# catid/longhair

Measured on AMD Instinct MI355X. Metric: GB/s of input data encoded+decoded, device-resident, per GPU and whole node, higher is better.
Workload: dtype u8

## Files before the change

### longhair_amd/csrc/codec.cpp

```cpp
#include <hip/hip_runtime.h>

#include <algorithm>
#include <atomic>
#include <cstdio>
#include <cstdlib>
#include <cstring>
#include <map>
#include <memory>
#include <mutex>
#include <stdexcept>
#include <thread>
#include <string>
#include <vector>

#include "../../include/cauchy_256.h"
#include "../../include/cauchy_256_batch.h"
#include "field.hpp"
#include "jit.hpp"
#include "host_codec.hpp"
#include "kernels.hpp"

namespace lh {

enum { kOk = 0, kInvalid = -1, kNoDevice = -2, kHipError = -3 };
// ... 136 lines not shown
    static constexpr int kDropinSlots = 4;
    DropinSlot dropin[kDropinSlots];
    std::mutex pipe_mu;
    hipStream_t pipe_stream[3] = {nullptr, nullptr, nullptr};
    hipEvent_t pipe_meta_ev = nullptr;
    DevBuf pipe_blocks[3], pipe_out[3];
    DevBuf pipe_rows, pipe_rows0, pipe_status;
    HostPinned pipe_meta;
};

static std::mutex g_devices_mu;
static std::map<int, std::unique_ptr<Device>> g_devices;

static int current_device(Device **out) {
    int id = 0;
    int count = 0;
    if (hipGetDeviceCount(&count) != hipSuccess || count <= 0)
        return fail(kNoDevice, "longhair_amd: no HIP device available (the codec has no CPU path)");
    LH_HIP(hipGetDevice(&id));
    std::lock_guard<std::mutex> g(g_devices_mu);
    auto &slot = g_devices[id];
    if (!slot) {
        std::unique_ptr<Device> d(new Device());
        d->id = id;
        const Field &F = Field::get();
        LH_HIP(hipMalloc(&d->gf_exp, 512));
        LH_HIP(hipMalloc(&d->gf_log, 256 * sizeof(int16_t)));
        LH_HIP(hipMemcpy(d->gf_exp, F.exp, 512, hipMemcpyHostToDevice));
        LH_HIP(hipMemcpy(d->gf_log, F.log, 256 * sizeof(int16_t), hipMemcpyHostToDevice));
        LH_HIP(hipDeviceGetAttribute(&d->cus, hipDeviceAttributeMultiprocessorCount, id));
        d->jump2 = jump_table2_usable(id);
        slot = std::move(d);
    }
    *out = slot.get();
    return kOk;
}

static bool capturing(hipStream_t st) {
    hipStreamCaptureStatus cs = hipStreamCaptureStatusNone;
    if (hipStreamIsCapturing(st, &cs) != hipSuccess) {
        (void)hipGetLastError();
        return false;
    }
    return cs != hipStreamCaptureStatusNone;
}

static int capture_growth_error(const char *what) {
    return fail(kHipError, std::string("longhair_amd: the ") + what +
                               " must grow while the stream is being captured; reserve it before capture with "
                               "cauchy_256_batch_prepare_stream(k, m, bytes, max_stripes, stream) or an "
                               "uncaptured call of the same size on that stream");
}

static int device_generator(Device *d, int k, int m, const uint8_t **out, const uint8_t **points = nullptr,
                            hipStream_t st = nullptr) {
    std::lock_guard<std::mutex> g(d->mu);
    auto it = d->generators.find({k, m});
    if (it == d->generators.end()) {
        if (capturing(st)) return capture_growth_error("generator matrix");
        std::vector<uint8_t> G = generator_matrix(k, m);
        std::vector<uint8_t> xs, ys;
        const bool pts = cauchy_points(k, m, xs, ys);
        if (pts) {
            G.insert(G.end(), xs.begin(), xs.end());
            G.insert(G.end(), ys.begin(), ys.end());
        }
        uint8_t *p = nullptr;
        LH_HIP(hipMalloc(&p, G.size()));
        LH_HIP(hipMemcpy(p, G.data(), G.size(), hipMemcpyHostToDevice));
        it = d->generators.emplace(std::make_pair(k, m), std::make_pair(p, pts)).first;
    }
    *out = it->second.first;
    if (points) *points = it->second.second ? it->second.first + (size_t)k * m : nullptr;
    return kOk;
}

static int zero_page(Device *d, size_t bytes, const uint8_t **out, hipStream_t st = nullptr) {
    std::lock_guard<std::mutex> g(d->mu);
    if (d->zero.size < bytes) {
        if (capturing(st)) return capture_growth_error("zero page");
        uint8_t *p = nullptr;
        LH_HIP(hipMalloc(&p, bytes));
        LH_HIP(hipMemsetAsync(p, 0, bytes, nullptr));
        LH_HIP(hipStreamSynchronize(nullptr));
        if (d->zero.ptr) d->retired.push_back(d->zero.ptr);
        d->zero.ptr = p;
        d->zero.size = bytes;
    }
    *out = d->zero.ptr;
    return kOk;
}

static int workspace(Device *d, hipStream_t st, size_t plan_bytes, size_t work_bytes, Workspace **out) {
    std::lock_guard<std::mutex> g(d->mu);
    Workspace &w = d->ws[st];
    if ((plan_bytes > w.plan.size || work_bytes > w.work.size) && capturing(st))
        return capture_growth_error("per-stream decode workspace");
    LH_HIP(w.plan.reserve(plan_bytes, st));
    if (work_bytes) LH_HIP(w.work.reserve(work_bytes, st));
    *out = &w;
    return kOk;
}

static long long jit_blocks(const JitConfig &cfg, int stripes) {
    const long long waves = cfg.spw ? (stripes + cfg.spw - 1) / cfg.spw : (long long)stripes * cfg.wps;
    long long blocks = (waves + 3) / 4;
    return blocks;
}
static long long jit_encode_blocks(const JitConfig &cfg, int stripes) {
    const long long waves = cfg.spw ? (stripes + cfg.spw - 1) / cfg.spw : (long long)stripes * cfg.wps;
    return (waves + cfg.enc_wpb - 1) / cfg.enc_wpb;
}
static int generic_word(int sub) {
    if (sub >= 4) return 4;
    if (sub >= 2) return 2;
    return 1;
}

static const JitKernels *jit_lookup(Device *d, const JitConfig &cfg, bool allow_compile, std::string *err,
                                    bool *hard) {
    const JitMode mode = allow_compile ? batch_jit_mode() : JitMode::kCached;
    bool failed = false;
    const JitKernels *jk = d->jit.get(cfg, err, mode, &failed);
    *hard = !jk && failed && mode == JitMode::kBlocking;
    return jk;
}
// ... 111 lines not shown

enum { kFormStrided = 1, kFormFamily = 2, kFormTable = 4 };
static void shape_configs(int k, int m, int bytes, bool decode, int forms, std::vector<JitConfig> *out) {
    JitConfig cfg, c;
    if (jit_config_for(k, m, bytes, decode, &cfg)) {
        if (forms & kFormStrided) out->push_back(cfg);
        if ((forms & kFormFamily) && !cfg.family && jit_family_config_for(k, m, bytes, &c, decode)) out->push_back(c);
        if ((forms & kFormTable) && jit_ptr_config_for(k, m, bytes, decode, &c)) out->push_back(c);
    } else if (jit_win_config_for(k, m, bytes, &cfg, decode)) {
        if (forms & kFormStrided) out->push_back(cfg);
        if ((forms & kFormTable) && jit_win_ptr_config_for(k, m, bytes, &c, decode)) out->push_back(c);
    }
}

static void note_jit_launch(const char *kernel, const Route &r, const Blocks &b) {
    char name[64];
    std::snprintf(name, sizeof name, "%s%s", kernel, b.table ? "(pointer table)" : r.cfg.family ? "(family)" : "");
    note_launch(name);
}

static int launch_jit_encode(const Route &r, int bytes, int stripes, Blocks in, Blocks out, hipStream_t st) {
    long long blocks = jit_encode_blocks(r.cfg, stripes);
    if (r.cfg.family) {
        const long long spw = 64 / ((bytes / 8 + 7) / 8);
        blocks = ((stripes + spw - 1) / spw + r.cfg.enc_wpb - 1) / r.cfg.enc_wpb;
    }
    if (blocks > 0x7FFFFFFF) return fail(kInvalid, "batch too large");
    int n = stripes, bb = bytes;
    void *args[] = {(void *)&in.p, &in.stride, (void *)&out.p, &out.stride, &n, &bb};
    const unsigned lds = in.table ? 0 : r.jk->dyn_lds;
    LH_HIP(hipModuleLaunchKernel(r.jk->encode, (unsigned)blocks, 1, 1, 64u * (unsigned)r.cfg.enc_wpb, 1, 1, lds, st,
                                 args, nullptr));
    note_jit_launch("lh_jit_encode", r, in);
    return kOk;
}

static int launch_jit_encode_win(const Route &r, int m, int bytes, int stripes, Blocks in, Blocks out, hipStream_t st) {
    const long long blocks = (long long)stripes * (r.cfg.sub / (64 * r.cfg.W));
    if (blocks > 0x7FFFFFFF) return fail(kInvalid, "batch too large");
    const unsigned threads = 64u * (unsigned)((m + r.cfg.rows_per_wave - 1) / r.cfg.rows_per_wave);
    int n = stripes, bb = bytes;
    void *args[] = {(void *)&in.p, &in.stride, (void *)&out.p, &out.stride, &n, &bb};
    LH_HIP(hipModuleLaunchKernel(r.jk->encode_win, (unsigned)blocks, 1, 1, threads, 1, 1, 0, st, args, nullptr));
    note_jit_launch("lh_jit_encode_win", r, in);
    return kOk;
}

static int launch_jit_decode_fused(Device *d, const Route &r, int bytes, int stripes, Blocks blk, uint8_t *d_rows,
                                   int8_t *d_status, hipStream_t st) {
    const long long blocks = jit_blocks(r.cfg, stripes);
    if (blocks > 0x7FFFFFFF) return fail(kInvalid, "batch too large");
    const uint8_t *zero = nullptr;
    if (int rc = zero_page(d, (size_t)bytes, &zero, st)) return rc;
    const uint8_t *gexp = d->gf_exp;
    const int16_t *glog = d->gf_log;
    int n = stripes, bb = bytes;
    void *args[] = {(void *)&blk.p, &blk.stride, (void *)&d_rows, (void *)&d_status, (void *)&zero,
                    (void *)&gexp, (void *)&glog, &n, &bb};
    const unsigned lds = blk.table ? 0 : r.jk->dyn_lds;
    LH_HIP(hipModuleLaunchKernel(r.jk->decode_fused, (unsigned)blocks, 1, 1, 256, 1, 1, lds, st, args, nullptr));
    note_jit_launch("lh_jit_decode_fused", r, blk);
    return kOk;
}

static int launch_jit_decode(Device *d, const Route &r, int bytes, int stripes, Blocks blk, const Workspace *w,
                             long long plan_stride, hipStream_t st) {
    const long long blocks = jit_blocks(r.cfg, stripes);
    if (blocks > 0x7FFFFFFF) return fail(kInvalid, "batch too large");
    const uint8_t *zero = nullptr;
    if (int rc = zero_page(d, (size_t)bytes, &zero, st)) return rc;
    const uint8_t *plan = w->plan.ptr;
    int n = stripes;
    void *args[] = {(void *)&blk.p, &blk.stride, (void *)&plan, &plan_stride, (void *)&zero, &n};
    LH_HIP(hipModuleLaunchKernel(r.jk->decode, (unsigned)blocks, 1, 1, 256, 1, 1, 0, st, args, nullptr));
    note_jit_launch("lh_jit_decode", r, blk);
    return kOk;
}

static size_t plan_order_offset(int stripes, long long plan_stride) {
    return ((size_t)stripes * (size_t)plan_stride + 15) & ~(size_t)15;
}
static size_t plan_workspace_bytes(int k, int m, int e_max, int stripes) {
    return plan_order_offset(stripes, PlanView::bytes(k, m, e_max)) + (size_t)stripes * sizeof(int);
}

static int launch_jit_decode_wide(Device *d, const Route &r, int k, int m, int e_max, int bytes, int stripes,
                                  Blocks blk, const Workspace *w, long long plan_stride, hipStream_t st) {
    const long long blocks = (long long)stripes * (r.cfg.sub / (64 * r.cfg.W));
    if (blocks > 0x7FFFFFFF) return fail(kInvalid, "batch too large");
    const uint8_t *zero = nullptr;
    if (int rc = zero_page(d, (size_t)bytes, &zero, st)) return rc;
    const unsigned threads = 64u * (unsigned)((m + r.cfg.rows_per_wave - 1) / r.cfg.rows_per_wave);
    const uint8_t *plan = w->plan.ptr;
    int n = stripes, bb = bytes;
    void *args[] = {(void *)&blk.p, &blk.stride, (void *)&plan, &plan_stride, (void *)&zero, &n, &bb};
    LH_HIP(hipModuleLaunchKernel(r.jk->decode_wide, (unsigned)blocks, 1, 1, threads, 1, 1, 0, st, args, nullptr));
    note_jit_launch("lh_jit_decode_wide", r, blk);
    InverseArgs ia{};
    set_blocks(ia, blk);
    ia.plan = plan;
    ia.plan_stride = plan_stride;
    ia.k = k;
    ia.m = m;
    ia.e_max = e_max;
    ia.bytes = bytes;
    ia.stripes = stripes;
    ia.order = (int *)(w->plan.ptr + plan_order_offset(stripes, plan_stride));
    LH_HIP(launch_inverse(ia, st));
    return kOk;
}

// ... 975 lines not shown
```

### longhair_amd/csrc/jit.cpp

```cpp
#include "jit.hpp"

#include <hip/hiprtc.h>
#include <dlfcn.h>
#include <sys/stat.h>
#include <unistd.h>
#include <utime.h>

#include <algorithm>
#include <cstdio>
#include <cstdlib>
#include <cstring>
#include <deque>
#include <functional>
#include <sstream>
#include <thread>

#include "field.hpp"

extern "C" const char lh_jit_source[];
extern "C" const char lh_inv_jump_source[];

namespace lh {

namespace {
// ... 456 lines not shown
    if (c.win) {
        std::string tok;
        for (char ch : c.defines + " ") {
            if (ch == ' ' || ch == ',') {
                const size_t eq = tok.find('=');
                if (!tok.empty()) os << "#define " << (eq == std::string::npos ? tok : tok.substr(0, eq) + " " + tok.substr(eq + 1)) << "\n";
                tok.clear();
            } else {
                tok += ch;
            }
        }
        os << win_source_for(c);
        return os.str();
    }
    {
        std::string tok;
        for (char ch : c.defines + " ") {
            if (ch == ' ' || ch == ',') {
                const size_t eq = tok.find('=');
                if (!tok.empty()) os << "#define " << (eq == std::string::npos ? tok : tok.substr(0, eq) + " " + tok.substr(eq + 1)) << "\n";
                tok.clear();
            } else {
                tok += ch;
            }
        }
    }
    if (c.family) {
        os << "#define LH_FAMILY 1\n#define LH_K " << c.k << "\n#define LH_M " << c.m
           << "\n#define LH_BYTES 1024\n#define LH_SUB 128\n#define LH_W 8\n#define LH_NCH 16\n#define LH_SPW 4"
              "\n#define LH_WPS 1\n#ifndef LH_LDS\n#define LH_LDS 1\n#endif\n#ifndef LH_CPS\n#define LH_CPS "
           << c.cps << "\n#endif\n#define LH_ROLE " << c.role << "\n#define LH_DEC_PLAIN 0\n";
    } else {
    os << "#define LH_K " << c.k << "\n#define LH_M " << c.m << "\n#define LH_BYTES " << c.bytes
       << "\n#define LH_SUB " << c.sub << "\n#define LH_W " << c.W << "\n#define LH_NCH " << c.nch
       << "\n#define LH_SPW " << (c.spw ? c.spw : 1) << "\n#define LH_WPS " << (c.wps ? c.wps : 1) << "\n";
    if (c.ptr) os << "#define LH_PTR 1\n#define LH_BUF 0\n";
    if (c.lds) os << "#ifndef LH_LDS\n#define LH_LDS 1\n#endif\n";
    if (c.cps > 1 && !c.ptr) os << "#ifndef LH_CPS\n#define LH_CPS " << c.cps << "\n#endif\n";
    if (c.role) os << "#define LH_ROLE " << c.role << "\n#define LH_DEC_PLAIN " << c.plain << "\n";
    }
    const std::vector<uint8_t> g = generator_matrix(c.k, c.m);
    os << "static constexpr unsigned char LH_BM[" << c.m << "][" << c.k << "][8] = {";
    for (int r = 0; r < c.m; ++r) {
        os << "{";
        for (int x = 0; x < c.k; ++x) {
            const uint64_t bm = bitmatrix(g[(size_t)r * c.k + x]);
            os << "{";
            for (int y = 0; y < 8; ++y) os << (unsigned)((bm >> (8 * y)) & 0xFF) << (y < 7 ? "," : "");
            os << "}" << (x + 1 < c.k ? "," : "");
        }
        os << "}" << (r + 1 < c.m ? "," : "");
    }
    os << "};\n";
    os << "#define LH_G_INIT {";
    for (int r = 0; r < c.m; ++r) {
        os << "{";
        for (int x = 0; x < c.k; ++x) os << (unsigned)g[(size_t)r * c.k + x] << (x + 1 < c.k ? "," : "");
        os << "}" << (r + 1 < c.m ? "," : "");
    }
    os << "}\n";
    os << lh_jit_source;
    return os.str();
}

JitCache::Key JitCache::key_of(const JitConfig &cfg) {
    return Key(cfg.k, cfg.m, (cfg.win || cfg.family) ? 0 : cfg.bytes, cfg.W, cfg.defines + (cfg.family ? "|family" : ""),
               cfg.lds * 1000000000 + cfg.ptr * 100000000 + (cfg.role + 3 * cfg.plain) * 10000000 +
                   cfg.win_split * 1000000 + cfg.win * 100000 + cfg.win_lds * 10000 +
                   cfg.rows_per_wave * 100 + cfg.win_pf);
}

const JitKernels *JitCache::peek(const JitConfig &cfg) {
    std::lock_guard<std::mutex> g(mu_);
    auto it = cache_.find(key_of(cfg));
    return it == cache_.end() ? nullptr : &it->second;
}

static const char *kOpts[] = {"--offload-arch=gfx950", "-O3", "-std=c++17", "-mllvm", "-enable-gvn-memdep=false",
                              "-mllvm", "-enable-load-pre=false"};

static uint64_t fnv1a(const std::string &s, uint64_t h = 1469598103934665603ull) {
    for (unsigned char ch : s) h = (h ^ ch) * 1099511628211ull;
    return h;
}

static std::string cache_dir() {
    if (const char *d = std::getenv("LONGHAIR_AMD_CACHE_DIR")) return d;
    Dl_info info;
    if (dladdr((void *)&fnv1a, &info) && info.dli_fname) {
        std::string p = info.dli_fname;
        const size_t slash = p.rfind('/');
        if (slash != std::string::npos) {
            std::string d = p.substr(0, slash) + "/jit_cache";
            mkdir(d.c_str(), 0755);
            if (access(d.c_str(), W_OK) == 0) return d;
        }
    }
    if (const char *home = std::getenv("HOME")) {
        std::string d = std::string(home) + "/.cache";
        mkdir(d.c_str(), 0755);
        d += "/longhair_amd";
        mkdir(d.c_str(), 0755);
        return d;
    }
    return "";
}

static std::string cache_path(const std::string &src) {
    std::string key = src;
    for (const char *o : kOpts) key += std::string("\n") + o;
    static const std::string ver = [] {
        int major = 0, minor = 0;
        (void)hiprtcVersion(&major, &minor);
// ... 304 lines not shown
```

### longhair_amd/csrc/jit_codec.hip

```cpp

#ifndef LH_K
#define LH_K 4
#define LH_M 2
#define LH_BYTES 64
#define LH_SUB 8
#define LH_W 8
#define LH_NCH 1
#define LH_SPW 64
#define LH_WPS 0
static constexpr unsigned char LH_BM[LH_M][LH_K][8] = {
    {{1, 2, 4, 8, 16, 32, 64, 128}, {1, 2, 4, 8, 16, 32, 64, 128},
     {1, 2, 4, 8, 16, 32, 64, 128}, {1, 2, 4, 8, 16, 32, 64, 128}},
    {{1, 2, 4, 8, 16, 32, 64, 128}, {2, 4, 8, 16, 32, 64, 128, 135},
     {3, 6, 12, 24, 48, 96, 192, 7}, {4, 8, 16, 32, 64, 128, 135, 137}}};
#define LH_G_INIT {{1, 1, 1, 1}, {1, 2, 3, 4}}
#include <hip/hip_runtime.h>
#endif

#define LH_NW ((LH_W + 3) / 4)


struct lh_word {
    unsigned int v[LH_NW];
};

#ifndef LH_NT
#define LH_NT 1
#endif
typedef unsigned int lh_u32x2 __attribute__((ext_vector_type(2)));
typedef unsigned int lh_u32x3 __attribute__((ext_vector_type(3)));
typedef unsigned int lh_u32x4 __attribute__((ext_vector_type(4)));

__device__ __forceinline__ lh_word lh_load(const unsigned char *p) {
    lh_word w;
#if LH_NT && LH_W == 16
    const lh_u32x4 v = __builtin_nontemporal_load((const lh_u32x4 *)p);
    w.v[0] = v.x; w.v[1] = v.y; w.v[2] = v.z; w.v[3] = v.w;
#elif LH_NT && LH_W == 12
    const lh_u32x3 v = __builtin_nontemporal_load((const lh_u32x3 *)p);
    w.v[0] = v.x; w.v[1] = v.y; w.v[2] = v.z;
#elif LH_NT && LH_W == 8
    const lh_u32x2 v = __builtin_nontemporal_load((const lh_u32x2 *)p);
    w.v[0] = v.x; w.v[1] = v.y;
#elif LH_NT && LH_W == 4
    w.v[0] = __builtin_nontemporal_load((const unsigned int *)p);
#else
#pragma unroll
    for (int i = 0; i < LH_NW; ++i) w.v[i] = 0;
    __builtin_memcpy(&w.v[0], p, LH_W);
#endif
    return w;
}

#ifndef LH_NT_ST
#define LH_NT_ST LH_NT
#endif
#ifndef LH_BUF
#define LH_BUF 1
#endif
#ifndef LH_PTR
#define LH_PTR 0
#endif
#if LH_PTR && LH_BUF
#error "LH_PTR: scattered blocks are addressed by 64-bit pointers (LH_BUF 0)"
#endif
#ifndef LH_NT_DEC
#define LH_NT_DEC 0
#endif
// ... 1171 lines not shown

template <int PF, class PREP>
__device__ __forceinline__ void lh_decode_body(const lh_lane &l, long long wave, unsigned char *__restrict__ blocks,
                                               long long stripe_stride, lh_plan_regs &pr,
                                               const unsigned char *__restrict__ zero_page, int stripes,
                                               const PREP &prep) {
    const lh_dsrc S = lh_make_dsrc(l, wave, blocks, stripe_stride, zero_page, stripes);
    lh_word v[LH_M][8];
    {
        lh_word ring[PF][8];
        lh_dec_issue<PF>(ring, pr, S);
        prep(pr);
        lh_dec_phase_a<PF>(v, ring, pr, S);
    }
#if LH_BUF
    lh_dec_phase_b(v, pr, blocks + l.stripe * stripe_stride + l.p, l.last, S, S.lbase - l.p);
#elif LH_PTR
    lh_dec_phase_b(v, pr, nullptr, l.last, S, l.p);
#else
    lh_dec_phase_b(v, pr, blocks + l.stripe * stripe_stride + l.p, l.last, S, 0);
#endif
}

__device__ __forceinline__ void lh_decode_wave(long long wave, unsigned char *__restrict__ blocks,
                                               long long stripe_stride, const unsigned char *__restrict__ plan,
                                               long long plan_stride, const unsigned char *__restrict__ zero_page,
                                               int stripes) {
    const lh_lane l = lh_map_lane(stripes, wave);
    if (!l.active) return;
    const unsigned char *pl = plan + l.stripe * plan_stride;
    lh_plan_regs pr;
    pr.e = pl[0];
    if (pr.e == 0) return;
    lh_load_packed(pr.srcw, pl + LH_P_SRC);
    lh_load_packed(pr.recw, pl + LH_P_REC);
    lh_load_packed(pr.coefw, pl + LH_P_COEF);
    lh_load_packed(pr.outw, pl + LH_P_OUT);
    lh_decode_body<LH_PF_DEC>(l, wave, blocks, stripe_stride, pr, zero_page, stripes, lh_no_prep());
}

#if LH_ROLE == 0 || (LH_ROLE == 2 && (LH_DEC_PLAIN || !(LH_EMAX <= 4 && LH_NCH <= 64 && LH_K <= 64)))
extern "C" __global__ void __launch_bounds__(256)
lh_jit_decode(unsigned char *__restrict__ blocks, long long stripe_stride,
              const unsigned char *__restrict__ plan, long long plan_stride,
              const unsigned char *__restrict__ zero_page, int stripes) {
    LH_WAVE_LOOP(stripes) { lh_decode_wave(lh_w, blocks, stripe_stride, plan, plan_stride, zero_page, stripes); }
}
#endif

#if LH_EMAX <= 4 && LH_NCH <= 64 && LH_K <= 64
#define LH_FUSED 1
#undef LH_DWPB
#define LH_DWPB 4
static constexpr unsigned char LH_GRAW[LH_M][LH_K] = LH_G_INIT;
#define LH_P4(n) (((n) + 3) / 4 * 4)
#define LH_SR (2 * LH_P4(LH_K) + LH_P4(LH_M))
#define LH_NRW ((LH_K + LH_NCH - 1) / LH_NCH)
#define LH_STRIPE_LANES (LH_NCH >= 64 ? ~0ull : ((1ull << (LH_NCH & 63)) - 1))

struct lh_gct {
    static constexpr int nch = LH_NCH, nrw = LH_NRW, maxrw = LH_NRW;
    static constexpr unsigned long long lanes = LH_STRIPE_LANES;
};

template <class G>
__device__ __forceinline__ void lh_fused_rows(const G &g, const lh_lane &l, int c, const unsigned char *__restrict__ rows,
                                              unsigned int (&rowv)[G::maxrw]) {
    const unsigned char *grow = rows + l.stripe * LH_K;
#pragma unroll
    for (int t = 0; t < G::maxrw; ++t) {
        const int i = c + t * g.nch;
        rowv[t] = (l.active && t < g.nrw && i < LH_K) ? (unsigned int)grow[i] : 0u;
    }
}

struct lh_fused_solve {
    unsigned int rs[LH_EMAX], rr[LH_EMAX], er[LH_EMAX];
    unsigned char *grow;
    const unsigned char *gexp;
    const short *glog;
    const unsigned char *gmat;
    int c;
    __device__ __forceinline__ void operator()(lh_plan_regs &pr) const;
};

template <class G>
__device__ __forceinline__ bool lh_fused_plan(const G &g, const lh_lane &l, int c, int sl, unsigned char *scr,
                                              const unsigned int (&rowv)[G::maxrw],
                                              unsigned char *__restrict__ rows, signed char *__restrict__ status,
                                              lh_fused_solve &sv, lh_plan_regs &pr) {
    unsigned char *lrows = scr;
    unsigned char *lsrc = scr + LH_P4(LH_K);
    unsigned char *lrec = lsrc + LH_P4(LH_K);
    unsigned char *grow = rows + l.stripe * LH_K;
    for (int q = c; q < (LH_P4(LH_K) + LH_P4(LH_M)) / 4; q += g.nch) ((unsigned int *)lsrc)[q] = 0xFFFFFFFFu;
    bool bad = false;
#pragma unroll
    for (int t = 0; t < G::maxrw; ++t) {
        const int i = c + t * g.nch;
        if (t >= g.nrw || i >= LH_K) continue;
        const unsigned int r = rowv[t];
        lrows[i] = (unsigned char)r;
        if (r < LH_K) lsrc[r] = (unsigned char)i;
        else if (r < LH_K + LH_M) lrec[r - LH_K] = (unsigned char)i;
        else bad = true;
    }
    for (int i = c; i < LH_K; i += g.nch) {
        const unsigned int r = lrows[i];
        if (r < LH_K + LH_M && (r < LH_K ? lsrc[r] : lrec[r - LH_K]) != i) bad = true;
    }
    const unsigned long long lanes_bad = __ballot(bad);
    const unsigned long long my = g.lanes << (sl * g.nch);
    const bool invalid = (lanes_bad & my) != 0;
    unsigned long long rcvmask = 0, ermask = 0;
#pragma unroll
    for (int t = 0; t < G::maxrw; ++t) {
        if (t >= g.nrw) break;
        const int i = c + t * g.nch;
        const bool isrcv = (i < LH_K) && (lrows[i] >= LH_K);
        const bool iser = (i < LH_K) && (lsrc[i] == 0xFF);
        rcvmask |= ((__ballot(isrcv) >> (sl * g.nch)) & g.lanes) << (t * g.nch);
        ermask |= ((__ballot(iser) >> (sl * g.nch)) & g.lanes) << (t * g.nch);
    }
    const int nr = __builtin_popcountll(rcvmask);
    unsigned int rs[LH_EMAX], rr[LH_EMAX], er[LH_EMAX];
#pragma unroll
    for (int q = 0; q < LH_EMAX; ++q) {
        rs[q] = rcvmask ? (unsigned int)__builtin_ctzll(rcvmask) : 0u;
        er[q] = ermask ? (unsigned int)__builtin_ctzll(ermask) : 0u;
        rcvmask &= rcvmask - 1;
        ermask &= ermask - 1;
        rr[q] = (unsigned int)lrows[rs[q]] - LH_K;
    }
    if (invalid || nr > LH_EMAX) {
        if (c == 0 && status) status[l.stripe] = -1;
        return false;
    }
    if (c == 0 && status) status[l.stripe] = 0;
    pr.e = nr;
    if (nr == 0) return false;
#pragma unroll
    for (int q = 0; q < LH_EMAX; ++q) { sv.rs[q] = rs[q]; sv.rr[q] = rr[q]; sv.er[q] = er[q]; }
    sv.grow = grow;
    sv.c = c;
#pragma unroll
    for (int q = 0; q < LH_NSRC; ++q) pr.srcw[q] = ((const unsigned int *)lsrc)[q];
#pragma unroll
    for (int q = 0; q < LH_NREC; ++q) pr.recw[q] = ((const unsigned int *)lrec)[q];
    return true;
}

template <int n> struct lh_perms;
template <> struct lh_perms<0> { static constexpr int cnt = 1; static constexpr int p[1][1] = {{0}}; };
template <> struct lh_perms<1> { static constexpr int cnt = 1; static constexpr int p[1][1] = {{0}}; };
template <> struct lh_perms<2> { static constexpr int cnt = 2; static constexpr int p[2][2] = {{0, 1}, {1, 0}}; };
template <> struct lh_perms<3> {
    static constexpr int cnt = 6;
    static constexpr int p[6][3] = {{0, 1, 2}, {0, 2, 1}, {1, 0, 2}, {1, 2, 0}, {2, 0, 1}, {2, 1, 0}};
};

template <int N>
__device__ __forceinline__ void lh_inv_adj(const unsigned int (&A)[N][N], unsigned int (&Ainv)[N][N],
                                           const unsigned char *gexp, const short *glog) {
    int L[N][N];
#pragma unroll
    for (int i = 0; i < N; ++i)
#pragma unroll
        for (int j = 0; j < N; ++j) L[i][j] = glog[A[i][j]];
    constexpr int M = N - 1;
    unsigned int C[N][N];
#pragma unroll
    for (int i = 0; i < N; ++i) {
        if (i > 0) {
#pragma unroll
            for (int j = 0; j < N; ++j) asm volatile("" : "+v"(C[i - 1][j]));
#pragma unroll
            for (int r = 0; r < N; ++r)
#pragma unroll
                for (int c = 0; c < N; ++c) asm volatile("" : "+v"(L[r][c]));
        }
#pragma unroll
        for (int j = 0; j < N; ++j) {
            unsigned int c = 0;
#pragma unroll
            for (int q = 0; q < lh_perms<M>::cnt; ++q) {
                int sum = 0;
                bool zero = false;
#pragma unroll
                for (int t = 0; t < M; ++t) {
                    const int r = t < i ? t : t + 1;
                    const int cc0 = lh_perms<M>::p[q][t];
                    const int cc = cc0 < j ? cc0 : cc0 + 1;
                    sum += L[r][cc];
                    zero = zero || A[r][cc] == 0u;
                }
                c ^= zero ? 0u : (unsigned int)gexp[sum];
            }
            C[i][j] = c;
        }
    }
    int LC[N][N];
#pragma unroll
    for (int i = 0; i < N; ++i)
#pragma unroll
        for (int j = 0; j < N; ++j) LC[i][j] = glog[C[i][j]];
    unsigned int det = 0;
#pragma unroll
    for (int j = 0; j < N; ++j) det ^= (A[0][j] && C[0][j]) ? (unsigned int)gexp[L[0][j] + LC[0][j]] : 0u;
    const int ninv = 255 - glog[det];
#pragma unroll
    for (int i = 0; i < N; ++i)
#pragma unroll
        for (int j = 0; j < N; ++j) Ainv[i][j] = C[j][i] ? (unsigned int)gexp[LC[j][i] + ninv] : 0u;
}

__device__ __forceinline__ void lh_fused_solve::operator()(lh_plan_regs &pr) const {
    const int nr = pr.e;
    unsigned int A[LH_EMAX][LH_EMAX], I[LH_EMAX][LH_EMAX];
#pragma unroll
    for (int i = 0; i < LH_EMAX; ++i)
#pragma unroll
        for (int j = 0; j < LH_EMAX; ++j)
            A[i][j] = (i < nr && j < nr) ? gmat[rr[i] * LH_K + er[j]] : (i == j ? 1u : 0u);
    lh_inv_adj<LH_EMAX>(A, I, gexp, glog);
#pragma unroll
    for (int i = 0; i < LH_EMAX; ++i)
#pragma unroll
        for (int j = 0; j < LH_EMAX; ++j) asm volatile("" : "+v"(I[i][j]));
#pragma unroll
    for (int q = 0; q < LH_NCOEF; ++q) pr.coefw[q] = 0;
#pragma unroll
    for (int i = 0; i < LH_EMAX; ++i)
#pragma unroll
        for (int r = 0; r < LH_M; ++r) {
            unsigned int v = 0;
#pragma unroll
            for (int j = 0; j < LH_EMAX; ++j) if (j < nr && rr[j] == (unsigned int)r) v = I[i][j];
            const int idx = i * LH_M + r;
            pr.coefw[idx / 4] |= v << (8 * (idx % 4));
        }
#pragma unroll
    for (int q = 0; q < LH_NOUT; ++q) pr.outw[q] = 0;
#pragma unroll
    for (int i = 0; i < LH_EMAX; ++i) pr.outw[i / 4] |= rs[i] << (8 * (i % 4));
    if (c == 0)
#pragma unroll
        for (int i = 0; i < LH_EMAX; ++i) if (i < nr) grow[rs[i]] = (unsigned char)er[i];
#pragma unroll
    for (int q = 0; q < LH_NCOEF; ++q) asm volatile("" : "+v"(pr.coefw[q]));
#pragma unroll
    for (int q = 0; q < LH_NOUT; ++q) asm volatile("" : "+v"(pr.outw[q]));
}

#if LH_LDS
#ifndef LH_LDS_REC_FIRST
#define LH_LDS_REC_FIRST 0
#endif
#ifndef LH_LDS_NT_DEC
#define LH_LDS_NT_DEC 1
#endif
#define LH_SR_SRC LH_P4(LH_K)
#define LH_SR_REC (2 * LH_P4(LH_K))
template <int X>
struct lh_dmoff {
    using D = lh_dcol<X, LH_LDS_REC_FIRST>;
    static constexpr int v = D::rec ? LH_SR_REC + D::r : LH_SR_SRC + D::x;
};
struct lh_dldsrc {
#if LH_PTR
    const unsigned long long *pt;
    int prow[LH_LQ];
    int joff[LH_LQ];
#else
    __amdgpu_buffer_rsrc_t rs;
    int joff[LH_LQ];
#endif
    int jsc[LH_LQ];
    const unsigned char *scr;
    unsigned char *ring;
    template <int X>
    __device__ __forceinline__ void slots(unsigned (&sv)[LH_LQ]) const {
#pragma unroll
        for (int q = 0; q < LH_LQ; ++q) {
            const unsigned b = scr[(jsc[q] & 0x7FFFFFFF) + lh_dmoff<X>::v];
            sv[q] = jsc[q] < 0 ? 0xFFu : b;
        }
    }
    __device__ __forceinline__ void issue(const unsigned (&sv)[LH_LQ], int slot) const {
#pragma unroll
        for (int q = 0; q < LH_LQ; ++q)
#if LH_PTR
            lh_dma16<LH_LDS_NT_DEC>((const unsigned char *)pt[prow[q] + (sv[q] == 0xFFu ? LH_K : (int)sv[q])] + joff[q],
                                    ring + slot * (LH_LQ * 1024) + q * 1024);
#else
            __builtin_amdgcn_raw_ptr_buffer_load_lds(
                rs, (__attribute__((address_space(3))) void *)(ring + slot * (LH_LQ * 1024) + q * 1024), 16,
                sv[q] == 0xFFu ? (int)0x80000000 : joff[q] + (int)sv[q] * LH_BYTES, 0, 0, LH_LDS_NT_DEC ? 2 : 0);
#endif
    }
};
#ifndef LH_LDG
#define LH_LDG (LH_LD > 2 ? 2 : 1)
#endif
#if LH_LDG < 1 || LH_LDG >= LH_LD
// ... 59 lines not shown
        if (i < e) {
            lh_word o[8];
#pragma unroll
            for (int y = 0; y < 8; ++y)
#pragma unroll
                for (int q = 0; q < LH_NW; ++q) o[y].v[q] = 0;
#pragma unroll
            for (int t = 7; t >= 0; --t) {
                if (t != 7) {
                    lh_word t7;
#pragma unroll
                    for (int q = 0; q < LH_NW; ++q) t7.v[q] = lh_x3(o[0].v[q], o[1].v[q], o[2].v[q]) ^ o[7].v[q];
#pragma unroll
                    for (int y = 0; y < 7; ++y) o[y] = o[y + 1];
                    o[7] = t7;
                }
#pragma unroll
                for (int r = 0; r < LH_M; ++r) {
                    const int idx = i * LH_M + r;
                    const unsigned int mask =
                        (unsigned int)((int)(pr.coefw[idx / 4] << (31 - (8 * (idx % 4) + t))) >> 31);
#pragma unroll
                    for (int y = 0; y < 8; ++y)
#pragma unroll
                        for (int q = 0; q < LH_NW; ++q) o[y].v[q] = lh_xand(o[y].v[q], v[r][y].v[q], mask);
                }
#if LH_PIN_WORDS & 2
                lh_pin8w(o);
#else
                lh_pin8(o);
#endif
            }
            unsigned char *d = dst((int)LH_BYTE(pr.outw, i));
#pragma unroll
            for (int y = 0; y < 8; ++y) {
                lh_word w = o[y];
                if constexpr (VL != 8) {
                    const lh_word f = lh_funnel<VL>(lh_row_shr1(w.v[0]), lh_row_shr1(w.v[1]), w.v[0], w.v[1]);
                    w.v[0] = last ? f.v[0] : w.v[0];
                    w.v[1] = last ? f.v[1] : w.v[1];
                }
                lh_store(d + y * sub, w);
                asm volatile("" ::: "memory");
            }
        }
    }
}
template <class DST>
__device__ __forceinline__ void lh_fused_out(const lh_word (&v)[LH_M][8], const lh_plan_regs &pr, bool last, DST dst) {
    lh_fused_out_g<LH_VLAST>(v, pr, last, LH_SUB, dst);
}
__device__ __forceinline__ void lh_fused_wave_lds(const lh_lane &l, long long wave, int c, int sl, bool work,
                                                  const unsigned char *scr, unsigned char *__restrict__ blocks,
                                                  long long stripe_stride, int stripes, const lh_fused_solve &sv,
                                                  lh_plan_regs &pr, const unsigned char *zero_page) {
    __shared__ __attribute__((aligned(16))) unsigned char lh_dring[LH_DWPB][LH_LD * LH_LQ * 1024 + LH_LPAD];
    const int lane = threadIdx.x & 63;
    const long long s0 = (long long)__builtin_amdgcn_readfirstlane((int)wave) * LH_SPW;
    if (s0 >= stripes) return;
    const int nst = (int)((stripes - s0) < LH_SPW ? (stripes - s0) : LH_SPW);
    const unsigned long long wm = __ballot(work);
    if (wm == 0) return;
    lh_dldsrc S;
#if LH_PTR
    __shared__ unsigned long long lh_dpt[LH_DWPB][LH_SPW * (LH_K + 1)];
    unsigned long long *prow = lh_dpt[threadIdx.x >> 6];
    __builtin_amdgcn_fence(__ATOMIC_RELEASE, "wavefront");
    __builtin_amdgcn_wave_barrier();
    if (sl < nst) {
        const unsigned long long *t = (const unsigned long long *)(blocks + (s0 + sl) * stripe_stride);
        for (int x = c; x <= LH_K; x += LH_NCH)
            prow[sl * (LH_K + 1) + x] = x < LH_K ? t[x] : (unsigned long long)zero_page;
    }
    __builtin_amdgcn_fence(__ATOMIC_RELEASE, "wavefront");
    __builtin_amdgcn_wave_barrier();
    __builtin_amdgcn_fence(__ATOMIC_ACQUIRE, "wavefront");
    S.pt = prow;
#else
    (void)zero_page;
    S.rs = __builtin_amdgcn_make_buffer_rsrc(blocks + s0 * stripe_stride, 0, (int)(nst * stripe_stride), 0x00020000);
#endif
    S.scr = scr;
    S.ring = lh_dring[(int)(threadIdx.x >> 6)];
#pragma unroll
    for (int q = 0; q < LH_LQ; ++q) {
        int j = 64 * q + lane;
        if (j >= nst * (LH_BYTES / 16)) j = nst * (LH_BYTES / 16) - 1;
        const int js = j / (LH_BYTES / 16);
#if LH_PTR
        S.prow[q] = js * (LH_K + 1);
        S.joff[q] = (j - js * (LH_BYTES / 16)) * 16;
#else
        S.joff[q] = js * (int)stripe_stride + (j - js * (LH_BYTES / 16)) * 16;
#endif
        S.jsc[q] = js * LH_SR | (((wm >> (js * LH_NCH)) & 1ull) ? 0 : (int)0x80000000);
    }
    asm volatile("s_waitcnt lgkmcnt(0)" ::: "memory");
    lh_decode_lds_prologue(S);
    if (work) sv(pr);
    lh_word v[LH_M][8];
#pragma unroll
    for (int r = 0; r < LH_M; ++r)
#pragma unroll
        for (int y = 0; y < 8; ++y)
#pragma unroll
            for (int i = 0; i < LH_NW; ++i) v[r][y].v[i] = 0;
    const int lo = (sl < LH_SPW ? sl : LH_SPW - 1) * LH_BYTES + 8 * c;
    int lo8 = lo + 8;
    asm volatile("" : "+v"(lo8));
    lh_unroll_decode_lds<0>::run(v, S, lo, lo8);
    if (!work) return;
#if LH_PTR
    lh_fused_out(v, pr, l.last, [&](int slot) {
        return (unsigned char *)S.pt[sl * (LH_K + 1) + slot] + (l.last ? LH_SUB - 8 : 8 * c);
    });
#else
    unsigned char *base = blocks + l.stripe * stripe_stride + (l.last ? LH_SUB - 8 : 8 * c);
    lh_fused_out(v, pr, l.last, [&](int slot) { return base + (long long)slot * LH_BYTES; });
#endif
}
#endif

#ifndef LH_DEC_LB
#define LH_DEC_LB 1
#endif
template <int PF>
__device__ __forceinline__ void lh_fused_body(unsigned char *__restrict__ blocks, long long stripe_stride,
                                              unsigned char *__restrict__ rows, signed char *__restrict__ status,
                                              const unsigned char *__restrict__ zero_page,
                                              const unsigned char *__restrict__ gf_exp,
                                              const short *__restrict__ gf_log, int stripes) {
    __shared__ unsigned char gexp[1024];
    __shared__ short glog[256];
    __shared__ unsigned char gmat[LH_M * LH_K];
    __shared__ __attribute__((aligned(16))) unsigned char scratch[LH_DWPB][LH_SPW > 0 ? LH_SPW : 1][LH_SR];
    for (int i = threadIdx.x; i < 256; i += blockDim.x) {
#pragma unroll
        for (int q = 0; q < 4; ++q) gexp[i + 256 * q] = gf_exp[(i + 256 * q) % 255];
        glog[i] = gf_log[i];
    }
    for (int i = threadIdx.x; i < LH_M * LH_K; i += blockDim.x) gmat[i] = LH_GRAW[i / LH_K][i % LH_K];
    __syncthreads();
    const int wid = threadIdx.x >> 6;
    LH_WAVE_LOOP(stripes) {
        const lh_lane l = lh_map_lane(stripes, lh_w);
        const int lane = threadIdx.x & 63;
        const int sl = lane / LH_NCH;
        const int c = lane - sl * LH_NCH;
        lh_plan_regs pr;
        lh_fused_solve sv;
        sv.gexp = gexp;
        sv.glog = glog;
        sv.gmat = gmat;
        unsigned int rowv[lh_gct::maxrw];
        lh_fused_rows(lh_gct(), l, c, rows, rowv);
#if LH_LDS
        const bool work = l.active && lh_fused_plan(lh_gct(), l, c, sl, &scratch[wid][sl][0], rowv, rows, status, sv, pr);
        lh_fused_wave_lds(l, lh_w, c, sl, work, &scratch[wid][0][0], blocks, stripe_stride, stripes, sv, pr, zero_page);
#else
        if (l.active && lh_fused_plan(lh_gct(), l, c, sl, &scratch[wid][sl][0], rowv, rows, status, sv, pr))
            lh_decode_body<PF>(l, lh_w, blocks, stripe_stride, pr, zero_page, stripes, sv);
#endif
    }
}

#if (LH_ROLE == 0 || (LH_ROLE == 2 && !LH_DEC_PLAIN)) && !LH_FAMILY
extern "C" __global__ void __launch_bounds__(64 * LH_DWPB, LH_DEC_LB)
lh_jit_decode_fused(unsigned char *__restrict__ blocks, long long stripe_stride, unsigned char *__restrict__ rows,
                    signed char *__restrict__ status, const unsigned char *__restrict__ zero_page,
                    const unsigned char *__restrict__ gf_exp, const short *__restrict__ gf_log, int stripes) {
    lh_fused_body<LH_PF_DEC>(blocks, stripe_stride, rows, status, zero_page, gf_exp, gf_log, stripes);
}
#endif

#if LH_FAMILY && LH_ROLE == 2 && LH_LDS && !LH_PTR
#define LH_FNRW 8
#define LH_FSPW (64 / ((LH_K + LH_FNRW - 1) / LH_FNRW))
#define LH_FRS (4 * 1024 + 16)
struct lh_grt {
    int nch, nrw;
    unsigned long long lanes;
    static constexpr int maxrw = LH_FNRW;
};
struct lh_dfam {
    int bytes, sub, nch, spw, cch;
};
struct lh_fdsrc {
    __amdgpu_buffer_rsrc_t rs;
    int joff[4], jsc[4];
    int bytes;
    const unsigned char *scr;
    unsigned char *ring;
    template <int X>
    __device__ __forceinline__ void slots(unsigned (&sv)[4]) const {
#pragma unroll
        for (int q = 0; q < 4; ++q) {
            const unsigned b = scr[(jsc[q] & 0x7FFFFFFF) + lh_dmoff<X>::v];
            sv[q] = jsc[q] < 0 ? 0xFFu : b;
        }
    }
    __device__ __forceinline__ void issue(const unsigned (&sv)[4], int slot) const {
#pragma unroll
        for (int q = 0; q < 4; ++q) {
            int off = slot * LH_FRS + q * 1024;
            asm volatile("" : "+s"(off));
            __builtin_amdgcn_raw_ptr_buffer_load_lds(
                rs, (__attribute__((address_space(3))) void *)(ring + off), 16,
                sv[q] == 0xFFu ? (int)0x80000000 : joff[q] + (int)sv[q] * bytes, 0, 0, LH_LDS_NT_DEC ? 2 : 0);
        }
    }
};
template <int C, int N>
__device__ __forceinline__ void lh_fdslots(const lh_fdsrc &S, unsigned (&sv)[LH_LDG][4]) {
    if constexpr (N > 0 && C < LH_DCOLS) {
        S.slots<C>(sv[LH_LDG - N]);
        lh_fdslots<C + 1, N - 1>(S, sv);
    }
}
template <int C, int N>
__device__ __forceinline__ void lh_fdissue(const lh_fdsrc &S, const unsigned (&sv)[LH_LDG][4]) {
    if constexpr (N > 0 && C < LH_DCOLS) {
        S.issue(sv[LH_LDG - N], C % LH_LD);
        lh_fdissue<C + 1, N - 1>(S, sv);
    }
// ... 5 lines not shown
        const int S = (b * R) & 7;
        const lh_u32x2a x = *(const lh_u32x2a *)(slot + ad[b] + ((b * R) & ~7));
        if (S == 0) {
            d[b].v[0] = x.x;
            d[b].v[1] = x.y;
        } else {
            const lh_u32x2a y = *(const lh_u32x2a *)(slot + ad[b] + 8 + ((b * R) & ~7));
            if (S == 2) d[b] = lh_funnel<2>(x.x, x.y, y.x, y.y);
            else if (S == 4) d[b] = lh_funnel<4>(x.x, x.y, y.x, y.y);
            else d[b] = lh_funnel<6>(x.x, x.y, y.x, y.y);
        }
    }
}
template <int X, int R>
struct lh_unroll_dfam {
    __device__ __forceinline__ static void run(lh_word (&v)[LH_M][8], const lh_fdsrc &S, const int (&ad)[8]) {
        if constexpr (X < LH_DCOLS) {
            constexpr int issued = (LH_LD + LH_LDG * (X / LH_LDG)) < LH_DCOLS ? (LH_LD + LH_LDG * (X / LH_LDG)) : LH_DCOLS;
            constexpr int ahead = issued - 1 - X;
            unsigned sv[4];
            if constexpr (LH_LDG == 1 && X + LH_LD < LH_DCOLS) S.slots<(X + LH_LD < LH_DCOLS ? X + LH_LD : 0)>(sv);
            constexpr bool refill = LH_LDG > 1 && (X + 1) % LH_LDG == 0 && LH_LD + X + 1 - LH_LDG < LH_DCOLS;
            unsigned svg[LH_LDG][4];
            if constexpr (refill) lh_fdslots<LH_LD + X + 1 - LH_LDG, LH_LDG>(S, svg);
            lh_wait_vmcnt<4 * ahead>();
            asm volatile("" ::: "memory");
            lh_word d[8];
            lh_dfam_col<R>(d, S.ring + (X % LH_LD) * LH_FRS, ad);
            lh_dcombine<X, LH_LDS_REC_FIRST>(v, d);
            lh_dopaque(v);
            if constexpr (LH_LDG == 1 && X + LH_LD < LH_DCOLS) {
                asm volatile("s_waitcnt lgkmcnt(0)" ::: "memory");
                S.issue(sv, X % LH_LD);
            } else if constexpr (refill) {
                asm volatile("s_waitcnt lgkmcnt(0)" ::: "memory");
                lh_fdissue<LH_LD + X + 1 - LH_LDG, LH_LDG>(S, svg);
            }
            lh_unroll_dfam<X + 1, R>::run(v, S, ad);
        }
    }
};
template <int X = 0>
__device__ __forceinline__ void lh_dfam_prologue(const lh_fdsrc &S) {
    if constexpr (X < LH_LD && X < LH_DCOLS) {
        unsigned sv[4];
        S.slots<X>(sv);
        S.issue(sv, X);
        lh_dfam_prologue<X + 1>(S);
    }
}
template <int R>
__device__ __forceinline__ void lh_fused_wave_fam(const lh_dfam &F, const lh_lane &l, long long wave, int c, int sl, bool work,
                                                  const unsigned char *scr, unsigned char *__restrict__ blocks,
                                                  long long stripe_stride, int stripes, const lh_fused_solve &sv,
                                                  lh_plan_regs &pr, unsigned char *ring) {
    const int lane = threadIdx.x & 63;
    const long long s0 = (long long)__builtin_amdgcn_readfirstlane((int)wave) * F.spw;
    if (s0 >= stripes) return;
    const int nst = (int)((stripes - s0) < F.spw ? (stripes - s0) : F.spw);
    const unsigned long long wm = __ballot(work);
    if (wm == 0) return;
    lh_fdsrc S;
    S.rs = __builtin_amdgcn_make_buffer_rsrc(blocks + s0 * stripe_stride, 0, (int)(nst * stripe_stride), 0x00020000);
    S.bytes = F.bytes;
    S.scr = scr;
    S.ring = ring;
#pragma unroll
    for (int q = 0; q < 4; ++q) {
        const int j = 64 * q + lane;
        const int js = j / F.cch;
        const bool on = js < nst && ((wm >> (js * F.nch)) & 1ull);
        S.joff[q] = js * (int)stripe_stride + (j - js * F.cch) * 16;
        S.jsc[q] = on ? js * LH_SR : (int)0x80000000;
    }
    asm volatile("s_waitcnt lgkmcnt(0)" ::: "memory");
    lh_dfam_prologue(S);
    if (work) sv(pr);
    lh_word v[LH_M][8];
#pragma unroll
    for (int r = 0; r < LH_M; ++r)
#pragma unroll
        for (int y = 0; y < 8; ++y)
#pragma unroll
            for (int i = 0; i < LH_NW; ++i) v[r][y].v[i] = 0;
    const int lo = (sl < F.spw ? sl : F.spw - 1) * F.bytes + 8 * c;
    int ad[8];
#pragma unroll
    for (int b = 0; b < 8; ++b) ad[b] = lo + b * (F.sub - R);
    lh_unroll_dfam<0, R>::run(v, S, ad);
    if (!work) return;
    unsigned char *base = blocks + l.stripe * stripe_stride + (l.last ? F.sub - 8 : 8 * c);
    lh_fused_out_g<R == 0 ? 8 : R>(v, pr, l.last, F.sub, [&](int slot) { return base + (long long)slot * F.bytes; });
}
template <int R>
__device__ __forceinline__ void lh_dfam_body(const lh_dfam &F, const lh_grt &g, unsigned char *__restrict__ blocks,
                                             long long stripe_stride, unsigned char *__restrict__ rows,
                                             signed char *__restrict__ status, const unsigned char *gexp, const short *glog,
                                             const unsigned char *gmat, unsigned char (*scratch)[LH_FSPW][LH_SR],
                                             unsigned char *ring, int stripes) {
    const int wid = threadIdx.x >> 6, lane = threadIdx.x & 63;
    const int sl = lane / F.nch, c = lane - sl * F.nch;
    const long long nw = ((long long)stripes + F.spw - 1) / F.spw;
    const long long ws = (long long)gridDim.x * (blockDim.x >> 6);
    for (long long w = (lh_block_id() * blockDim.x + threadIdx.x) >> 6; w < nw; w += ws) {
        lh_lane l;
        l.stripe = w * F.spw + sl;
        l.active = sl < F.spw && l.stripe < stripes;
        l.last = c == F.nch - 1;
        l.p = 0;
        lh_plan_regs pr;
        lh_fused_solve sv;
        sv.gexp = gexp;
        sv.glog = glog;
        sv.gmat = gmat;
        unsigned int rowv[LH_FNRW];
        lh_fused_rows(g, l, c, rows, rowv);
        const bool work = l.active && lh_fused_plan(g, l, c, sl, &scratch[wid][sl][0], rowv, rows, status, sv, pr);
        lh_fused_wave_fam<R>(F, l, w, c, sl, work, &scratch[wid][0][0], blocks, stripe_stride, stripes, sv, pr, ring);
    }
}
extern "C" __global__ void __launch_bounds__(256, LH_DEC_LB)
lh_jit_decode_fused(unsigned char *__restrict__ blocks, long long stripe_stride, unsigned char *__restrict__ rows,
                    signed char *__restrict__ status, const unsigned char *__restrict__ zero_page,
                    const unsigned char *__restrict__ gf_exp, const short *__restrict__ gf_log, int stripes, int bytes) {
    (void)zero_page;
    __shared__ unsigned char gexp[1024];
    __shared__ short glog[256];
    __shared__ unsigned char gmat[LH_M * LH_K];
    __shared__ __attribute__((aligned(16))) unsigned char scratch[4][LH_FSPW][LH_SR];
    __shared__ __attribute__((aligned(16))) unsigned char lh_fdring[4][LH_LD * LH_FRS];
    for (int i = threadIdx.x; i < 256; i += blockDim.x) {
#pragma unroll
        for (int q = 0; q < 4; ++q) gexp[i + 256 * q] = gf_exp[(i + 256 * q) % 255];
        glog[i] = gf_log[i];
    }
    for (int i = threadIdx.x; i < LH_M * LH_K; i += blockDim.x) gmat[i] = LH_GRAW[i / LH_K][i % LH_K];
    __syncthreads();
    lh_dfam F;
    F.bytes = bytes;
    F.sub = bytes >> 3;
    F.nch = (F.sub + 7) >> 3;
    F.spw = 64 / F.nch;
    F.cch = bytes >> 4;
    lh_grt g;
    g.nch = F.nch;
    g.nrw = (LH_K + F.nch - 1) / F.nch;
    g.lanes = F.nch >= 64 ? ~0ull : ((1ull << F.nch) - 1);
    unsigned char *ring = lh_fdring[__builtin_amdgcn_readfirstlane((int)(threadIdx.x >> 6))];
    switch (F.sub & 7) {
        case 0: lh_dfam_body<0>(F, g, blocks, stripe_stride, rows, status, gexp, glog, gmat, scratch, ring, stripes); break;
        case 2: lh_dfam_body<2>(F, g, blocks, stripe_stride, rows, status, gexp, glog, gmat, scratch, ring, stripes); break;
        case 4: lh_dfam_body<4>(F, g, blocks, stripe_stride, rows, status, gexp, glog, gmat, scratch, ring, stripes); break;
        default: lh_dfam_body<6>(F, g, blocks, stripe_stride, rows, status, gexp, glog, gmat, scratch, ring, stripes); break;
    }
}
#endif

#endif
```

Before: 4776.

## Pack GF tables into one device blob and defer decode metadata writes

Precomputes the GF exp/log tables and generator matrix into a single contiguous device buffer next to the generator, so each fused-decode block loads them into LDS with one 16-byte vector copy per thread instead of per-element modulo loops and constant-array reads. It also moves the status and recovered-row writes out of the solve and planning phases into a separate meta step that runs just before output, which shortens the register live ranges around the solve. The cost is a larger per-(k,m) device allocation and a launch path that now looks up the generator on every decode call.

Result: no change. 4841, median of 6 (+1.4%).

```diff
diff --git a/longhair_amd/csrc/codec.cpp b/longhair_amd/csrc/codec.cpp
--- a/longhair_amd/csrc/codec.cpp
+++ b/longhair_amd/csrc/codec.cpp
@@ -212,19 +212,28 @@
                                "uncaptured call of the same size on that stream");
 }
 
+static size_t fused_tables_offset(int k, int m) { return ((size_t)k * m + (size_t)k + m + 15) & ~(size_t)15; }
+
 static int device_generator(Device *d, int k, int m, const uint8_t **out, const uint8_t **points = nullptr,
-                            hipStream_t st = nullptr) {
+                            hipStream_t st = nullptr, const uint8_t **fused = nullptr) {
     std::lock_guard<std::mutex> g(d->mu);
     auto it = d->generators.find({k, m});
     if (it == d->generators.end()) {
         if (capturing(st)) return capture_growth_error("generator matrix");
         std::vector<uint8_t> G = generator_matrix(k, m);
+        const size_t km = G.size();
         std::vector<uint8_t> xs, ys;
         const bool pts = cauchy_points(k, m, xs, ys);
         if (pts) {
             G.insert(G.end(), xs.begin(), xs.end());
             G.insert(G.end(), ys.begin(), ys.end());
         }
+        const Field &F = Field::get();
+        const size_t off = fused_tables_offset(k, m);
+        G.resize(off + 1536 + ((km + 15) & ~(size_t)15), 0);
+        for (int i = 0; i < 1024; ++i) G[off + i] = F.exp[i % 255];
+        std::memcpy(&G[off + 1024], F.log, 256 * sizeof(int16_t));
+        std::memcpy(&G[off + 1536], G.data(), km);
         uint8_t *p = nullptr;
         LH_HIP(hipMalloc(&p, G.size()));
         LH_HIP(hipMemcpy(p, G.data(), G.size(), hipMemcpyHostToDevice));
@@ -232,6 +241,7 @@
     }
     *out = it->second.first;
     if (points) *points = it->second.second ? it->second.first + (size_t)k * m : nullptr;
+    if (fused) *fused = it->second.first + fused_tables_offset(k, m);
     return kOk;
 }
 
@@ -449,11 +459,11 @@
     if (blocks > 0x7FFFFFFF) return fail(kInvalid, "batch too large");
     const uint8_t *zero = nullptr;
     if (int rc = zero_page(d, (size_t)bytes, &zero, st)) return rc;
-    const uint8_t *gexp = d->gf_exp;
-    const int16_t *glog = d->gf_log;
+    const uint8_t *G = nullptr, *tab = nullptr;
+    if (int rc = device_generator(d, r.cfg.k, r.cfg.m, &G, nullptr, st, &tab)) return rc;
     int n = stripes, bb = bytes;
     void *args[] = {(void *)&blk.p, &blk.stride, (void *)&d_rows, (void *)&d_status, (void *)&zero,
-                    (void *)&gexp, (void *)&glog, &n, &bb};
+                    (void *)&tab, &n, &bb};
     const unsigned lds = blk.table ? 0 : r.jk->dyn_lds;
     LH_HIP(hipModuleLaunchKernel(r.jk->decode_fused, (unsigned)blocks, 1, 1, 256, 1, 1, lds, st, args, nullptr));
     note_jit_launch("lh_jit_decode_fused", r, blk);
diff --git a/longhair_amd/csrc/jit.cpp b/longhair_amd/csrc/jit.cpp
--- a/longhair_amd/csrc/jit.cpp
+++ b/longhair_amd/csrc/jit.cpp
@@ -532,13 +532,6 @@
         os << "}" << (r + 1 < c.m ? "," : "");
     }
     os << "};\n";
-    os << "#define LH_G_INIT {";
-    for (int r = 0; r < c.m; ++r) {
-        os << "{";
-        for (int x = 0; x < c.k; ++x) os << (unsigned)g[(size_t)r * c.k + x] << (x + 1 < c.k ? "," : "");
-        os << "}" << (r + 1 < c.m ? "," : "");
-    }
-    os << "}\n";
     os << lh_jit_source;
     return os.str();
 }
diff --git a/longhair_amd/csrc/jit_codec.hip b/longhair_amd/csrc/jit_codec.hip
--- a/longhair_amd/csrc/jit_codec.hip
+++ b/longhair_amd/csrc/jit_codec.hip
@@ -13,7 +13,6 @@
      {1, 2, 4, 8, 16, 32, 64, 128}, {1, 2, 4, 8, 16, 32, 64, 128}},
     {{1, 2, 4, 8, 16, 32, 64, 128}, {2, 4, 8, 16, 32, 64, 128, 135},
      {3, 6, 12, 24, 48, 96, 192, 7}, {4, 8, 16, 32, 64, 128, 135, 137}}};
-#define LH_G_INIT {{1, 1, 1, 1}, {1, 2, 3, 4}}
 #include <hip/hip_runtime.h>
 #endif
 
@@ -1291,7 +1290,6 @@
 #define LH_FUSED 1
 #undef LH_DWPB
 #define LH_DWPB 4
-static constexpr unsigned char LH_GRAW[LH_M][LH_K] = LH_G_INIT;
 #define LH_P4(n) (((n) + 3) / 4 * 4)
 #define LH_SR (2 * LH_P4(LH_K) + LH_P4(LH_M))
 #define LH_NRW ((LH_K + LH_NCH - 1) / LH_NCH)
@@ -1315,12 +1313,14 @@
 
 struct lh_fused_solve {
     unsigned int rs[LH_EMAX], rr[LH_EMAX], er[LH_EMAX];
+    unsigned int erw;
     unsigned char *grow;
     const unsigned char *gexp;
     const short *glog;
     const unsigned char *gmat;
     int c;
-    __device__ __forceinline__ void operator()(lh_plan_regs &pr) const;
+    __device__ __forceinline__ void operator()(lh_plan_regs &pr);
+    __device__ __forceinline__ void meta(const lh_plan_regs &pr, signed char *__restrict__ status, long long stripe) const;
 };
 
 template <class G>
@@ -1375,7 +1375,7 @@
         if (c == 0 && status) status[l.stripe] = -1;
         return false;
     }
-    if (c == 0 && status) status[l.stripe] = 0;
+    if (c == 0 && status && nr == 0) status[l.stripe] = 0;
     pr.e = nr;
     if (nr == 0) return false;
 #pragma unroll
@@ -1453,7 +1453,7 @@
         for (int j = 0; j < N; ++j) Ainv[i][j] = C[j][i] ? (unsigned int)gexp[LC[j][i] + ninv] : 0u;
 }
 
-__device__ __forceinline__ void lh_fused_solve::operator()(lh_plan_regs &pr) const {
+__device__ __forceinline__ void lh_fused_solve::operator()(lh_plan_regs &pr) {
     const int nr = pr.e;
     unsigned int A[LH_EMAX][LH_EMAX], I[LH_EMAX][LH_EMAX];
 #pragma unroll
@@ -1482,13 +1482,22 @@
     for (int q = 0; q < LH_NOUT; ++q) pr.outw[q] = 0;
 #pragma unroll
     for (int i = 0; i < LH_EMAX; ++i) pr.outw[i / 4] |= rs[i] << (8 * (i % 4));
-    if (c == 0)
-#pragma unroll
-        for (int i = 0; i < LH_EMAX; ++i) if (i < nr) grow[rs[i]] = (unsigned char)er[i];
+    erw = 0;
+#pragma unroll
+    for (int i = 0; i < LH_EMAX; ++i) erw |= er[i] << (8 * i);
+    asm volatile("" : "+v"(erw));
 #pragma unroll
     for (int q = 0; q < LH_NCOEF; ++q) asm volatile("" : "+v"(pr.coefw[q]));
 #pragma unroll
     for (int q = 0; q < LH_NOUT; ++q) asm volatile("" : "+v"(pr.outw[q]));
+}
+__device__ __forceinline__ void lh_fused_solve::meta(const lh_plan_regs &pr, signed char *__restrict__ status,
+                                                     long long stripe) const {
+    if (c != 0) return;
+    if (status) status[stripe] = 0;
+#pragma unroll
+    for (int i = 0; i < LH_EMAX; ++i)
+        if (i < pr.e) grow[LH_BYTE(pr.outw, i)] = (unsigned char)(erw >> (8 * i));
 }
 
 #if LH_LDS
@@ -1654,8 +1663,9 @@
 }
 __device__ __forceinline__ void lh_fused_wave_lds(const lh_lane &l, long long wave, int c, int sl, bool work,
                                                   const unsigned char *scr, unsigned char *__restrict__ blocks,
-                                                  long long stripe_stride, int stripes, const lh_fused_solve &sv,
-                                                  lh_plan_regs &pr, const unsigned char *zero_page) {
+                                                  long long stripe_stride, int stripes, lh_fused_solve &sv,
+                                                  lh_plan_regs &pr, const unsigned char *zero_page,
+                                                  signed char *__restrict__ status) {
     __shared__ __attribute__((aligned(16))) unsigned char lh_dring[LH_DWPB][LH_LD * LH_LQ * 1024 + LH_LPAD];
     const int lane = threadIdx.x & 63;
     const long long s0 = (long long)__builtin_amdgcn_readfirstlane((int)wave) * LH_SPW;
@@ -1712,6 +1722,7 @@
     asm volatile("" : "+v"(lo8));
     lh_unroll_decode_lds<0>::run(v, S, lo, lo8);
     if (!work) return;
+    sv.meta(pr, status, l.stripe);
 #if LH_PTR
     lh_fused_out(v, pr, l.last, [&](int slot) {
         return (unsigned char *)S.pt[sl * (LH_K + 1) + slot] + (l.last ? LH_SUB - 8 : 8 * c);
@@ -1723,6 +1734,14 @@
 }
 #endif
 
+#define LH_TABN (1536 + (LH_M * LH_K + 15) / 16 * 16)
+__device__ __forceinline__ const unsigned char *lh_fused_tables(const unsigned char *__restrict__ gf_tab) {
+    __shared__ __attribute__((aligned(16))) unsigned char tab[LH_TABN];
+    if (threadIdx.x < LH_TABN / 16) ((uint4 *)tab)[threadIdx.x] = ((const uint4 *)gf_tab)[threadIdx.x];
+    __syncthreads();
+    return tab;
+}
+
 #ifndef LH_DEC_LB
 #define LH_DEC_LB 1
 #endif
@@ -1730,19 +1749,11 @@
 __device__ __forceinline__ void lh_fused_body(unsigned char *__restrict__ blocks, long long stripe_stride,
                                               unsigned char *__restrict__ rows, signed char *__restrict__ status,
                                               const unsigned char *__restrict__ zero_page,
-                                              const unsigned char *__restrict__ gf_exp,
-                                              const short *__restrict__ gf_log, int stripes) {
-    __shared__ unsigned char gexp[1024];
-    __shared__ short glog[256];
-    __shared__ unsigned char gmat[LH_M * LH_K];
+                                              const unsigned char *__restrict__ gf_tab, int stripes) {
     __shared__ __attribute__((aligned(16))) unsigned char scratch[LH_DWPB][LH_SPW > 0 ? LH_SPW : 1][LH_SR];
-    for (int i = threadIdx.x; i < 256; i += blockDim.x) {
-#pragma unroll
-        for (int q = 0; q < 4; ++q) gexp[i + 256 * q] = gf_exp[(i + 256 * q) % 255];
-        glog[i] = gf_log[i];
-    }
-    for (int i = threadIdx.x; i < LH_M * LH_K; i += blockDim.x) gmat[i] = LH_GRAW[i / LH_K][i % LH_K];
-    __syncthreads();
+    const unsigned char *gexp = lh_fused_tables(gf_tab);
+    const short *glog = (const short *)(gexp + 1024);
+    const unsigned char *gmat = gexp + 1536;
     const int wid = threadIdx.x >> 6;
     LH_WAVE_LOOP(stripes) {
         const lh_lane l = lh_map_lane(stripes, lh_w);
@@ -1758,10 +1769,13 @@
         lh_fused_rows(lh_gct(), l, c, rows, rowv);
 #if LH_LDS
         const bool work = l.active && lh_fused_plan(lh_gct(), l, c, sl, &scratch[wid][sl][0], rowv, rows, status, sv, pr);
-        lh_fused_wave_lds(l, lh_w, c, sl, work, &scratch[wid][0][0], blocks, stripe_stride, stripes, sv, pr, zero_page);
+        lh_fused_wave_lds(l, lh_w, c, sl, work, &scratch[wid][0][0], blocks, stripe_stride, stripes, sv, pr, zero_page, status);
 #else
         if (l.active && lh_fused_plan(lh_gct(), l, c, sl, &scratch[wid][sl][0], rowv, rows, status, sv, pr))
-            lh_decode_body<PF>(l, lh_w, blocks, stripe_stride, pr, zero_page, stripes, sv);
+            lh_decode_body<PF>(l, lh_w, blocks, stripe_stride, pr, zero_page, stripes, [&](lh_plan_regs &p) {
+                sv(p);
+                sv.meta(p, status, l.stripe);
+            });
 #endif
     }
 }
@@ -1770,8 +1784,8 @@
 extern "C" __global__ void __launch_bounds__(64 * LH_DWPB, LH_DEC_LB)
 lh_jit_decode_fused(unsigned char *__restrict__ blocks, long long stripe_stride, unsigned char *__restrict__ rows,
                     signed char *__restrict__ status, const unsigned char *__restrict__ zero_page,
-                    const unsigned char *__restrict__ gf_exp, const short *__restrict__ gf_log, int stripes) {
-    lh_fused_body<LH_PF_DEC>(blocks, stripe_stride, rows, status, zero_page, gf_exp, gf_log, stripes);
+                    const unsigned char *__restrict__ gf_tab, int stripes) {
+    lh_fused_body<LH_PF_DEC>(blocks, stripe_stride, rows, status, zero_page, gf_tab, stripes);
 }
 #endif
 
@@ -1883,8 +1897,9 @@
 template <int R>
 __device__ __forceinline__ void lh_fused_wave_fam(const lh_dfam &F, const lh_lane &l, long long wave, int c, int sl, bool work,
                                                   const unsigned char *scr, unsigned char *__restrict__ blocks,
-                                                  long long stripe_stride, int stripes, const lh_fused_solve &sv,
-                                                  lh_plan_regs &pr, unsigned char *ring) {
+                                                  long long stripe_stride, int stripes, lh_fused_solve &sv,
+                                                  lh_plan_regs &pr, unsigned char *ring,
+                                                  signed char *__restrict__ status) {
     const int lane = threadIdx.x & 63;
     const long long s0 = (long long)__builtin_amdgcn_readfirstlane((int)wave) * F.spw;
     if (s0 >= stripes) return;
@@ -1920,6 +1935,7 @@
     for (int b = 0; b < 8; ++b) ad[b] = lo + b * (F.sub - R);
     lh_unroll_dfam<0, R>::run(v, S, ad);
     if (!work) return;
+    sv.meta(pr, status, l.stripe);
     unsigned char *base = blocks + l.stripe * stripe_stride + (l.last ? F.sub - 8 : 8 * c);
     lh_fused_out_g<R == 0 ? 8 : R>(v, pr, l.last, F.sub, [&](int slot) { return base + (long long)slot * F.bytes; });
 }
@@ -1947,26 +1963,19 @@
         unsigned int rowv[LH_FNRW];
         lh_fused_rows(g, l, c, rows, rowv);
         const bool work = l.active && lh_fused_plan(g, l, c, sl, &scratch[wid][sl][0], rowv, rows, status, sv, pr);
-        lh_fused_wave_fam<R>(F, l, w, c, sl, work, &scratch[wid][0][0], blocks, stripe_stride, stripes, sv, pr, ring);
+        lh_fused_wave_fam<R>(F, l, w, c, sl, work, &scratch[wid][0][0], blocks, stripe_stride, stripes, sv, pr, ring, status);
     }
 }
 extern "C" __global__ void __launch_bounds__(256, LH_DEC_LB)
 lh_jit_decode_fused(unsigned char *__restrict__ blocks, long long stripe_stride, unsigned char *__restrict__ rows,
                     signed char *__restrict__ status, const unsigned char *__restrict__ zero_page,
-                    const unsigned char *__restrict__ gf_exp, const short *__restrict__ gf_log, int stripes, int bytes) {
+                    const unsigned char *__restrict__ gf_tab, int stripes, int bytes) {
     (void)zero_page;
-    __shared__ unsigned char gexp[1024];
-    __shared__ short glog[256];
-    __shared__ unsigned char gmat[LH_M * LH_K];
     __shared__ __attribute__((aligned(16))) unsigned char scratch[4][LH_FSPW][LH_SR];
     __shared__ __attribute__((aligned(16))) unsigned char lh_fdring[4][LH_LD * LH_FRS];
-    for (int i = threadIdx.x; i < 256; i += blockDim.x) {
-#pragma unroll
-        for (int q = 0; q < 4; ++q) gexp[i + 256 * q] = gf_exp[(i + 256 * q) % 255];
-        glog[i] = gf_log[i];
-    }
-    for (int i = threadIdx.x; i < LH_M * LH_K; i += blockDim.x) gmat[i] = LH_GRAW[i / LH_K][i % LH_K];
-    __syncthreads();
+    const unsigned char *gexp = lh_fused_tables(gf_tab);
+    const short *glog = (const short *)(gexp + 1024);
+    const unsigned char *gmat = gexp + 1536;
     lh_dfam F;
     F.bytes = bytes;
     F.sub = bytes >> 3;
```
